# lazytiger/pbrt-rs

Measured on AMD Instinct MI355X. Metric: Mrays/s, higher is better.
Workload: dtype f32

## Files before the change

pbrt-rs_amd/csrc/pbrt_hip.hip:

```cpp
#include <hip/hip_runtime.h>
#include "abi_guard.h"

#include <algorithm>
#include <cstdio>
#include <cstdlib>
#include <cstring>
#include <string>
#include <vector>

#include "host_envmap.h"
#include "host_wide.h"
#include "scene.h"
#include "trace.h"
#include "trace_persistent.h"
#include "trace_wide.h"
#include "trace_stackless.h"

using namespace pb;

static thread_local std::string g_create_error;



extern "C" int pbrt_hip_context_create(int device_id, PbrtHipContext** out) try {
// ... 15 lines not shown
        delete ctx;
        return PBRT_HIP_ERR_DEVICE;
    }
    hipDeviceProp_t prop;
    if (hipGetDeviceProperties(&prop, device_id) != hipSuccess) {
        g_create_error = "hipGetDeviceProperties failed";
        delete ctx;
        return PBRT_HIP_ERR_DEVICE;
    }
    ctx->n_cus = prop.multiProcessorCount;
    ctx->trace_log = std::getenv("PBRT_HIP_TRACE_LOG") != nullptr;
    if (hipStreamCreateWithFlags(&ctx->stream, hipStreamNonBlocking) != hipSuccess ||
        hipEventCreate(&ctx->ev0) != hipSuccess || hipEventCreate(&ctx->ev1) != hipSuccess ||
        hipMalloc((void**)&ctx->d_counters, 8 * sizeof(unsigned long long)) != hipSuccess ||
        hipMalloc((void**)&ctx->d_work_counter, kWorkCounters * sizeof(unsigned int)) != hipSuccess ||
        hipHostMalloc((void**)&ctx->h_counts, 2 * sizeof(unsigned long long), hipHostMallocDefault) != hipSuccess ||
        hipEventCreateWithFlags(&ctx->ev_sync, hipEventDisableTiming) != hipSuccess ||
        hipMemset(ctx->d_counters, 0, 8 * sizeof(unsigned long long)) != hipSuccess) {
        g_create_error = "stream / event creation failed";
        delete ctx;
        return PBRT_HIP_ERR_DEVICE;
    }
    *out = ctx;
    return PBRT_HIP_OK;
}
PB_ABI_CATCH

extern "C" void pbrt_hip_context_destroy(PbrtHipContext* ctx) {
    if (!ctx) return;
    (void)hipSetDevice(ctx->device);
    if (ctx->lost) {
// ... 1355 lines not shown
```

pbrt-rs_amd/csrc/render.hip:

```cpp
#include <hip/hip_runtime.h>
#include "abi_guard.h"

#include <algorithm>
#include <chrono>
#include <cstdio>
#include <cstdlib>
#include <cstring>
#include <string>
#include <thread>
#include <vector>

#include "scene.h"
#include "trace.h"
#include "wavefront.h"

using namespace pb;

extern "C" int pbrt_hip_render_device(PbrtHipScene* s, const PbrtCamera* camera, const PbrtRenderParams* params,
                                      float* d_film, PbrtRenderStats* stats) try {
    if (!s || !camera || !params || !d_film) return PBRT_HIP_ERR_INVALID;
    PB_ENTER(s->ctx);
    HIP_TRY(s->ctx, hipSetDevice(s->ctx->device));
    return wavefront_render(s, *camera, *params, d_film, stats);
}
// ... 650 lines not shown
    ps.two_level = s->d.bvh.instanced ? 1 : 0;
    ps.ray = buf.alloc<float4>(N * 6, &ok);
    ps.hit = buf.alloc<float4>(N * 6, &ok);
    ps.rng = buf.alloc<uint64_t>(N, &ok);
    ps.L = buf.alloc<float4>(N, &ok);
    ps.beta = buf.alloc<float4>(N, &ok);
    ps.nee_a = buf.alloc<float4>(N, &ok);
    ps.nee_f = buf.alloc<float4>(N, &ok);
    ps.nee_b = buf.alloc<float4>(N, &ok);
    ps.nee_light = buf.alloc<int>(N, &ok);
    ps.pfilm = buf.alloc<float2>(N, &ok);
    Queues q[2];
    for (int k = 0; k < 2; ++k) {
        q[k].trace = buf.alloc<uint32_t>(N * 3, &ok);
        q[k].shade = buf.alloc<uint32_t>(N, &ok);
        q[k].counts64 = buf.alloc<unsigned long long>(2, &ok);
        q[k].keys = nullptr;
        for (int a = 0; a < 3; ++a) {
            const float lo = s->d.bvh.root_min[a], hi = s->d.bvh.root_max[a];
            q[k].key_lo[a] = lo;
            q[k].key_inv[a] = hi > lo ? 1.0f / (hi - lo) : 0.0f;
        }
    }
    if (rp.ray_order < 0 || rp.ray_order > 1) return invalid("ray_order must be 0 (Morton order from the second bounce on) or 1 (queue order)");
    const bool sort_rays = rp.ray_order == 0 && rp.integrator == PBRT_INTEGRATOR_PATH;
    constexpr int sort_from = 2;
    uint32_t *sort_keys[2] = {nullptr, nullptr}, *sort_vals = nullptr;
    void* sort_tmp = nullptr;
    size_t sort_tmp_bytes = 0;
    if (sort_rays) {
        sort_keys[0] = buf.alloc<uint32_t>(N * 3, &ok);
// ... 124 lines not shown
    std::memcpy(cam.r2c, camera.raster_to_camera, 64);
    cam.lens_radius = camera.lens_radius;
    cam.focal_distance = camera.focal_distance;
    cam.shutter_open = camera.shutter_open;
    cam.shutter_close = camera.shutter_close;
    cam.kind = camera.kind;
    if (camera.kind < PBRT_CAMERA_PERSPECTIVE || camera.kind > PBRT_CAMERA_ENVIRONMENT) return invalid("unknown camera kind");

    ShadeConsts sc;
    sc.bvh = s->d.bvh;
    sc.materials = s->d.materials;
    sc.lights = s->d.lights;
    sc.n_lights = s->d.n_lights;
    sc.n_infinite = s->d.n_infinite;
    sc.infinite_ids = s->d.infinite_ids;
    sc.env_maps = s->d.env_maps;
    sc.distrib = (rp.light_strategy == 0 || s->d.n_lights == 1) ? s->d.light_distrib_uniform : s->d.light_distrib_power;
    if (rp.integrator == PBRT_INTEGRATOR_PATH && (rp.light_strategy < 0 || rp.light_strategy > 2))
        return invalid("path: light_strategy must be 0 (uniform), 1 (power) or 2 (spatial)");
    std::memcpy(sc.env_cond_func, s->d.env_cond_func, sizeof(sc.env_cond_func));
    std::memcpy(sc.env_cond_cdf, s->d.env_cond_cdf, sizeof(sc.env_cond_cdf));
    std::memcpy(sc.env_cond_int, s->d.env_cond_int, sizeof(sc.env_cond_int));
    std::memcpy(sc.env_marg_func, s->d.env_marg_func, sizeof(sc.env_marg_func));
    std::memcpy(sc.env_marg_cdf, s->d.env_marg_cdf, sizeof(sc.env_marg_cdf));
    sc.env_marg_int = s->d.env_marg_int;
    sc.world_radius = s->d.world_radius;
    sc.light_sample_prefix = d_prefix;
    sc.total_light_samples = prefix.back();
    sc.spatial = nullptr;
    sc.n_voxel[0] = sc.n_voxel[1] = sc.n_voxel[2] = 1;
    sc.mis_bool = ctx->count_traversal != 1 ? 1 : 0;
    if (rp.integrator == PBRT_INTEGRATOR_PATH && rp.light_strategy == 2 && s->d.n_lights > 1) {
        if (!s->d_spatial) {
            const float* mn = s->d.bvh.root_min;
            const float* mx = s->d.bvh.root_max;
            float diag[3] = {mx[0] - mn[0], mx[1] - mn[1], mx[2] - mn[2]};
            int ext = (diag[0] > diag[1] && diag[0] > diag[2]) ? 0 : (diag[1] > diag[2] ? 1 : 2);
            for (int i = 0; i < 3; ++i) s->spatial_voxels[i] = std::max(1, (int)std::round(diag[i] / diag[ext] * 64.0f));
            size_t n_voxels = (size_t)s->spatial_voxels[0] * s->spatial_voxels[1] * s->spatial_voxels[2];
            size_t floats = n_voxels * (size_t)(2 * s->d.n_lights + 2);
            if (floats > (1ull << 30)) return invalid("spatial light distribution: voxels x lights exceed 4 GB; use \"power\"");
            void* p = nullptr;
            HIP_TRY(ctx, hipMalloc(&p, floats * sizeof(float)));
            s->allocs.push_back(p);
            for (int i = 0; i < 3; ++i) sc.n_voxel[i] = s->spatial_voxels[i];
            hipLaunchKernelGGL(k_spatial_light_tables, dim3((unsigned)((n_voxels + 63) / 64)), dim3(64), 0, st, sc, (float*)p);
// ... 134 lines not shown
                    } else if (inst == 2) {
                        if (count_ref) PB_LAUNCH_BINARY(true, 2, false); else PB_LAUNCH_BINARY(false, 2, false);
                    } else if (inst == 1) {
                        if (count_ref) PB_LAUNCH_BINARY(true, 1, false); else PB_LAUNCH_BINARY(false, 1, false);
                    } else {
                        if (count_ref) PB_LAUNCH_BINARY(true, 0, false); else PB_LAUNCH_BINARY(false, 0, false);
                    }
#undef PB_LAUNCH_BINARY
#undef PB_LAUNCH_WIDE
#undef PB_LAUNCH_SPECIAL
                }
                RENDER_TRY(hipGetLastError());
                RENDER_TRY(hipEventRecord(e_t1, st));
            }
            int nxt = cur ^ 1;
            RENDER_TRY(hipMemsetAsync(q[nxt].counts64, 0, 2 * sizeof(unsigned long long), st));
            q[nxt].keys = (sort_rays && wavefront + 1 >= sort_from) ? sort_keys[0] : nullptr;
            if (direct)
{
                dim3 sg((n_shade + 255) / 256), sb(256);
                if (rp.integrator == PBRT_INTEGRATOR_DIRECT && s->glossy)
                    hipLaunchKernelGGL((k_shade_direct<PBRT_INTEGRATOR_DIRECT, true>), sg, sb, 0, st, sc, ps, ds, q[cur], q[nxt], pp, tiles, n_shade);
                else if (rp.integrator == PBRT_INTEGRATOR_DIRECT)
                    hipLaunchKernelGGL((k_shade_direct<PBRT_INTEGRATOR_DIRECT, false>), sg, sb, 0, st, sc, ps, ds, q[cur], q[nxt], pp, tiles, n_shade);
                else if (rp.integrator == PBRT_INTEGRATOR_WHITTED && s->glossy)
                    hipLaunchKernelGGL((k_shade_direct<PBRT_INTEGRATOR_WHITTED, true>), sg, sb, 0, st, sc, ps, ds, q[cur], q[nxt], pp, tiles, n_shade);
                else if (rp.integrator == PBRT_INTEGRATOR_WHITTED)
                    hipLaunchKernelGGL((k_shade_direct<PBRT_INTEGRATOR_WHITTED, false>), sg, sb, 0, st, sc, ps, ds, q[cur], q[nxt], pp, tiles, n_shade);
                else
                    hipLaunchKernelGGL((k_shade_direct<PBRT_INTEGRATOR_AO, false>), sg, sb, 0, st, sc, ps, ds, q[cur], q[nxt], pp, tiles, n_shade);
            }
            else {
                Queues qin = q[cur];
                if (sort_shade && wavefront >= 1 && n_shade >= (1u << 10)) {
                    hipLaunchKernelGGL(k_shade_sort_keys, dim3((n_shade + 255) / 256), dim3(256), 0, st, sc, ps, q[cur].shade, n_shade,
                                       pp.max_depth, shade_keys[0]);
                    size_t tb = shade_tmp_bytes;
                    if (pb::sort_pairs_u32(st, shade_tmp, &tb, shade_keys[0], shade_keys[1], q[cur].shade, shade_sorted, n_shade, 3) != 0 &&
                        rc == PBRT_HIP_OK) {
                        ctx->last_error = "rocPRIM radix sort failed";
                        rc = PBRT_HIP_ERR_DEVICE;
                    }
                    qin.shade = shade_sorted;
                }
                const dim3 sg((n_shade + 255) / 256), sb(256);
                if (bin_shade && wavefront >= 1 && s->glossy)
                    hipLaunchKernelGGL((k_shade<true, true>), sg, sb, 0, st, sc, ps, qin, q[nxt], pp, tiles, n_shade);
                else if (bin_shade && wavefront >= 1)
                    hipLaunchKernelGGL((k_shade<true, false>), sg, sb, 0, st, sc, ps, qin, q[nxt], pp, tiles, n_shade);
                else if (s->glossy)
                    hipLaunchKernelGGL((k_shade<false, true>), sg, sb, 0, st, sc, ps, qin, q[nxt], pp, tiles, n_shade);
                else
                    hipLaunchKernelGGL((k_shade<false, false>), sg, sb, 0, st, sc, ps, qin, q[nxt], pp, tiles, n_shade);
            }
            RENDER_TRY(hipGetLastError());
            RENDER_TRY(hipMemcpyAsync(ctx->h_counts, q[nxt].counts64, sizeof(counts), hipMemcpyDeviceToHost, st));
            RENDER_TRY(hipEventRecord(ctx->ev_sync, st));
            if (rc == PBRT_HIP_OK) {
                hipError_t qe;
                const auto spin_start = std::chrono::steady_clock::now();
                uint32_t polls = 0;
                while ((qe = hipEventQuery(ctx->ev_sync)) == hipErrorNotReady) {
                    if ((++polls & 0xfffu) == 0) {
                        const double waited = std::chrono::duration<double>(std::chrono::steady_clock::now() - spin_start).count();
                        if (waited > ctx->wavefront_deadline_s) {
                            ctx->last_error = "a wavefront did not finish within the deadline (hung kernel?)";
                            ctx->lost = true;
                            rc = PBRT_HIP_ERR_DEVICE;
                            break;
                        }
                        if (waited > 0.05) std::this_thread::yield();
                    }
                }
                if (rc == PBRT_HIP_OK) RENDER_TRY(qe);
            }
            counts[0] = ctx->h_counts[0];
            counts[1] = ctx->h_counts[1];
            if (n_trace > 0 && rc == PBRT_HIP_OK) {
                float ms = 0.0f;
                RENDER_TRY(hipEventElapsedTime(&ms, e_t0, e_t1));
                local.trace_ms += ms;
                local.trace_launches += 1;
                if (ctx->trace_log)
                    std::fprintf(stderr, "[pbrt_hip] k_trace: %u rays %.3f ms (%.0f Mrays/s)\n", n_trace, ms, n_trace / ms * 1e-3);
                ctx->trace_ms += ms;
                ctx->trace_launches += 1;
            }
            {
                uint64_t n_rays = counts[0] & 0xffffffffull, n_shadow = counts[0] >> 32;
                local.rays_closest += n_rays - n_shadow;
                local.rays_shadow += n_shadow;
                counts[0] = n_rays;
            }
            (void)first;
            first = false;
            wavefront += 1;
            cur = nxt;
        }
        if (li_mode) {
            hipLaunchKernelGGL(k_li_output, dim3((unsigned)((li->n + 255) / 256)), dim3(256), 0, st, ps, (uint32_t)li->n, li->d_rgb);
            RENDER_TRY(hipGetLastError());
            continue;
        }
        if (!box) {
            hipLaunchKernelGGL(k_film_splat, dim3((n_paths + 255) / 256), dim3(256), 0, st, ps, pp, tiles, d_film);
            RENDER_TRY(hipGetLastError());
            continue;
// ... 48 lines not shown
```

pbrt-rs_amd/csrc/scene.h:

```cpp
#pragma once
#include <atomic>
#include <hip/hip_runtime.h>

#include <algorithm>
#include <cmath>
#include <cstring>
#include <mutex>
#include <string>
#include <vector>

#include "../../include/pbrt_hip.h"
#include "trace.h"
#include "wide_bvh.h"

#define PB_LOCK(ctx) std::lock_guard<std::recursive_mutex> pb_lock_((ctx)->mu)
#define PB_ENTER(ctx)                                                                                              \
    PB_LOCK(ctx);                                                                                                  \
    if ((ctx)->lost) {                                                                                             \
        (ctx)->last_error = "context lost: an earlier call ran into the wavefront deadline; destroy the context";  \
        return PBRT_HIP_ERR_DEVICE;                                                                                \
    }

struct PbrtHipContext {
    std::recursive_mutex mu;
    int device = 0;
    hipStream_t stream = nullptr;
    hipEvent_t ev0 = nullptr, ev1 = nullptr;
    int n_cus = 0;
    std::string last_error;
    std::atomic<bool> lost{false};
    bool trace_log = false;
    double wavefront_deadline_s = 120.0;
    double trace_ms = 0.0;
    uint64_t trace_launches = 0;
    bool time_trace = true;
    int count_traversal = 0;
// ... 209 lines not shown
```

pbrt-rs_amd/csrc/wf_lights.h:

```cpp
#pragma once
#include "wf_microfacet.h"

namespace pb {

PB_DEV V3 sphere_through(V3 v) {
    return V3{1.0f * v.x + 0.0f * v.y + 0.0f * v.z, 0.0f * v.x + 1.0f * v.y + 0.0f * v.z, 0.0f * v.x + 0.0f * v.y + 1.0f * v.z};
}
PB_DEV float sphere_area(float radius) { return (360.0f * (kPi / 180.0f)) * radius * (radius - (-radius)); }
PB_DEV void sphere_light_sample(float cx, float cy, float cz, float radius, const Surf& sf, float u0, float u1, V3* p_o,
                                V3* err_o, V3* n_o, float* pdf_o) {
    V3 pc = V3{1.0f * 0.0f + 0.0f * 0.0f + 0.0f * 0.0f + cx, 0.0f * 0.0f + 1.0f * 0.0f + 0.0f * 0.0f + cy,
               0.0f * 0.0f + 0.0f * 0.0f + 1.0f * 0.0f + cz};
    V3 p_origin = offset_ray_origin(sf.p, sf.p_error, sf.n, pc - sf.p);
    if (len2(p_origin - pc) <= radius * radius) {
        float z = 1.0f - 2.0f * u0;
        float rr = __builtin_sqrtf(fmaxr(1.0f - z * z, 0.0f));
        float sp, cp;
        det_sincos(2.0f * kPi * u1, &sp, &cp);
        V3 obj = V3{rr * cp, rr * sp, z} * radius;
        V3 n = normalize(sphere_through(obj));
        obj = obj * (radius / length(obj));
        V3 oe = vabs(obj) * kGamma5;
        const float g3 = kGamma3;
        V3 p = V3{1.0f * obj.x + 0.0f * obj.y + 0.0f * obj.z + cx, 0.0f * obj.x + 1.0f * obj.y + 0.0f * obj.z + cy,
// ... 219 lines not shown
    for (int j = 0; j < n; ++j) func[j] = fmaxr(func[j], min_contrib);
    cdf[0] = 0.0f;
    for (int j = 1; j < n + 1; ++j) cdf[j] = cdf[j - 1] + func[j - 1] / (float)n;
    float func_int = cdf[n];
    if (func_int == 0.0f) {
        for (int j = 1; j < n + 1; ++j) cdf[j] = (float)j / (float)n;
    } else {
        for (int j = 1; j < n + 1; ++j) cdf[j] /= func_int;
    }
    func[2 * n + 1] = func_int;
}

template <class Bsdf>
PB_DEV int estimate_direct_emit(const ShadeConsts& sc, const PathState& ps, uint32_t p, const Surf& sf, const Frame& fr,
                                bool nonspecular, const Bsdf& bsdf, int light_num, float ul0, float ul1, float us0, float us1,
                                float pick_pdf, V3 beta) {
    if (!nonspecular) return 0;
    V3 wo = sf.wo;
    DevLight lt = sc.lights[light_num];
    V3 wi, li, p1, p1_err, p1_n;
    float light_pdf;
    light_sample_li(sc, sf, lt, ul0, ul1, &wi, &light_pdf, &li, &p1, &p1_err, &p1_n);
    int nee_flags = 0;
    V3 A = V3{0.0f, 0.0f, 0.0f};
    if (light_pdf > 0.0f && !is_black(li)) {
        V3 f;
        float scattering_pdf;
        bsdf_f_pdf(bsdf, fr, wo, wi, &f, &scattering_pdf);
        f = f * absdot(wi, fr.ns);
        if (!is_black(f)) {
            V3 origin = offset_ray_origin(sf.p, sf.p_error, sf.n, p1 - sf.p);
            V3 target = offset_ray_origin(p1, p1_err, p1_n, origin - p1);
            V3 d = target - origin;
            store_ray(ps, p, RS_SHADOW, origin, d, 1.0f - kShadowEpsilon);
// ... 70 lines not shown
            store_ray(ps, p, RS_MIS, o2, wi2, kInf);
            ps.nee_f[p] = make_float4(f2.x, f2.y, f2.z, weight);
            nee_flags |= PF_NEE_MIS;
            if (sc.mis_bool && lt.type != PBRT_LIGHT_DIFFUSE_AREA) nee_flags |= NEE_MIS_BOOL;
        }
    }
    if (nee_flags) {
        ps.nee_a[p] = make_float4(A.x, A.y, A.z, pick_pdf);
        ps.nee_b[p] = make_float4(beta.x, beta.y, beta.z, spdf);
        ps.nee_light[p] = light_num;
    }
    return nee_flags;
}

PB_DEV V3 estimate_direct_resolve(const ShadeConsts& sc, const PathState& ps, uint32_t p, int flags, float* pick_pdf,
                                  V3* beta_at_vertex) {
    float4 na = ps.nee_a[p], nf = ps.nee_f[p], nb = ps.nee_b[p];
    int light_id = ps.nee_light[p];
    V3 ld = V3{0.0f, 0.0f, 0.0f};
    if (flags & PF_NEE_SHADOW) {
        bool occluded = ps.hit[hit_index(ps, p, RS_SHADOW)].x != 0.0f;
        if (!occluded) ld = ld + V3{na.x, na.y, na.z};
    }
    if (flags & PF_NEE_MIS) {
        int hslot = __float_as_int(ps.hit[hit_index(ps, p, RS_MIS)].x);
        DevLight lt = sc.lights[light_id];
        V3 li = V3{0.0f, 0.0f, 0.0f};
        if (hslot >= 0) {
            int hl = lt.type == PBRT_LIGHT_DIFFUSE_AREA ? (__float_as_int(sc.bvh.tris[3 * (size_t)hslot + 2].w) & kPrimLightMask) - 1 : -2;
            if (hl == light_id) {
                float4 r0 = ps.ray[ray_index(ps, p, RS_MIS)], r1 = ps.ray[ray_index(ps, p, RS_MIS) + 1];
                V3 wi = V3{r0.w, r1.x, r1.y};
                float4 hb = ps.hit[hit_index(ps, p, RS_MIS)];
                V3 n = tri_interaction_normal(sc.bvh, hslot, hb.y, hb.z, hb.w);
                if (lt.two_sided || dot(n, -wi) > 0.0f) li = V3{lt.L[0], lt.L[1], lt.L[2]};
            }
        } else if (lt.type == PBRT_LIGHT_INFINITE) {
            if (lt.slot >= 0) {
                float4 r0 = ps.ray[ray_index(ps, p, RS_MIS)], r1 = ps.ray[ray_index(ps, p, RS_MIS) + 1];
                li = env_le(sc.env_maps[lt.slot], V3{r0.w, r1.x, r1.y});
            } else {
// ... 62 lines not shown
```

pbrt-rs_amd/csrc/wf_path.h:

```cpp
#pragma once
#include "wf_lights.h"

namespace pb {

PB_DEV uint32_t shade_key(const ShadeConsts& sc, const PathState& ps, uint32_t p, int max_depth) {
    int fb = __float_as_int(ps.beta[p].w);
    uint32_t key = 0;
    if ((fb & PF_ALIVE) && (fb >> 8) < max_depth) {
        const size_t hb = hit_index(ps, p, RS_CONT);
        int slot = __float_as_int(ps.hit[hb].x), inst = hit_instance(ps, hb);
        if (slot >= 0) {
            int mat = __float_as_int(sc.bvh.tris[3 * (size_t)slot + 2].z);
            if (sc.bvh.instanced && inst >= 0) {
                int over = __float_as_int(sc.bvh.instances[7 * (size_t)inst + 6].x);
                if (over >= 0) mat = over;
            }
            key = 1u + (uint32_t)sc.materials[mat].type;
        }
    }
    return key;
}
__global__ void k_shade_sort_keys(ShadeConsts sc, PathState ps, const uint32_t* __restrict__ shade_queue, uint32_t n, int max_depth,
                                  uint32_t* __restrict__ keys) {
    uint32_t i = blockIdx.x * blockDim.x + threadIdx.x;
    if (i >= n) return;
    keys[i] = shade_key(sc, ps, shade_queue[i], max_depth);
}

constexpr int shade_keys(bool glossy) { return glossy ? 8 : 6; }
template <int KEYS>
struct ShadeBins {
    uint32_t count[4][KEYS];
    uint32_t path[256];
};

#ifndef PB_SHADE_WAVES
#define PB_SHADE_WAVES 3
#endif
template <bool BIN, bool GLOSSY>
__global__ void __launch_bounds__(256, PB_SHADE_WAVES) k_shade(ShadeConsts sc, PathState ps, Queues qin, Queues qout, PassParams pp,
                                                 TileList tiles, uint32_t n_in) {
    constexpr int kShadeKeys = shade_keys(GLOSSY);
    uint32_t i = blockIdx.x * blockDim.x + threadIdx.x;
    bool active = i < n_in;
    uint32_t p = active ? qin.shade[i] : 0u;
    if (BIN) {
        __shared__ ShadeBins<kShadeKeys> bins;
        const int lane = threadIdx.x & 63, wave = threadIdx.x >> 6;
        const uint32_t key = active ? shade_key(sc, ps, p, pp.max_depth) : (uint32_t)(kShadeKeys - 1);
        uint32_t rank = 0;
#pragma unroll
        for (int k = 0; k < kShadeKeys; ++k) {
            const unsigned long long m = __ballot(key == (uint32_t)k);
            if (key == (uint32_t)k) rank = lane_prefix(m);
            if (lane == 0) bins.count[wave][k] = (uint32_t)__popcll(m);
        }
        __syncthreads();
        uint32_t before = 0;
        for (int k = 0; k < kShadeKeys; ++k)
            for (int w = 0; w < 4; ++w)
                before += ((uint32_t)k < key || ((uint32_t)k == key && w < wave)) ? bins.count[w][k] : 0u;
        bins.path[before + rank] = p;
        uint32_t n_active = 0;
        for (int k = 0; k < kShadeKeys - 1; ++k)
            for (int w = 0; w < 4; ++w) n_active += bins.count[w][k];
        __syncthreads();
        p = bins.path[threadIdx.x];
        active = threadIdx.x < n_active;
    }
    bool emit_cont = false, emit_mis = false, emit_shadow = false, mis_bool = false;

    uint32_t cell = 0;
    if (active) {
        float4 Lq = ps.L[p], bq = ps.beta[p];
        V3 L = V3{Lq.x, Lq.y, Lq.z};
        float eta_scale = Lq.w;
        V3 beta = V3{bq.x, bq.y, bq.z};
        int fb = __float_as_int(bq.w);
        int flags = fb & 0xff, bounces = fb >> 8;
        size_t rbase = ray_index(ps, p, RS_CONT), hbase = hit_index(ps, p, RS_CONT);

        if (flags & (PF_NEE_SHADOW | PF_NEE_MIS)) {
            float pick_pdf;
            V3 beta_v;
            V3 ld = estimate_direct_resolve(sc, ps, p, flags, &pick_pdf, &beta_v);
            ld = ld / pick_pdf;
            L = L + mulv(beta_v, ld);
            flags &= ~(PF_NEE_SHADOW | PF_NEE_MIS);
        }

        if (flags & PF_ALIVE) {
            flags &= ~PF_ALIVE;
            float4 r0 = ps.ray[rbase], r1 = ps.ray[rbase + 1];
            V3 rd = V3{r0.w, r1.x, r1.y};
            float4 h0 = ps.hit[hbase];
            int hslot = __float_as_int(h0.x);
            bool found = hslot >= 0;
            Surf sf;
            if (found) {
                sf = surface_from_hit(sc.bvh, hslot, hit_instance(ps, hbase), h0.y, h0.z, h0.w, rd);
                if (qout.keys) cell = ray_sort_cell(sf.p.x, sf.p.y, sf.p.z, qout.key_lo, qout.key_inv);
            }
            if (bounces == 0 || (flags & PF_SPECULAR_BOUNCE)) {
                if (found) {
                    L = L + mulv(beta, surface_le(sc, sf, -rd));
                } else {
                    for (int k = 0; k < sc.n_infinite; ++k) {
                        DevLight lt = sc.lights[sc.infinite_ids[k]];
                        V3 le = lt.slot >= 0 ? env_le(sc.env_maps[lt.slot], rd) : V3{lt.L[0], lt.L[1], lt.L[2]};
                        L = L + mulv(beta, le);
                    }
                }
            }
            if (found && bounces < pp.max_depth) {
                DevMaterial mat = sc.materials[sf.material];
                Samp sm = path_sampler(ps, pp, tiles, p);
                if (mat.type == PBRT_MAT_NONE) {
                    V3 o = offset_ray_origin(sf.p, sf.p_error, sf.n, rd);
                    store_ray(ps, p, RS_CONT, o, rd, kInf);
                    flags |= PF_ALIVE;
                    emit_cont = true;
                } else {
                    Frame fr = make_frame(sf);
                    V3 kd = V3{mat.kd[0], mat.kd[1], mat.kd[2]};
                    V3 kt = V3{mat.kt[0], mat.kt[1], mat.kt[2]};
                    V3 wo = -rd;
                    bool has_lobe;
                    bool nonspecular;
                    NsBsdf nsb;
                    if (GLOSSY) {
                        nsb = ns_bsdf(mat);
                        nonspecular = nsb.n > 0;
                        if (mat.type == PBRT_MAT_GLASS) has_lobe = !(is_black(kd) && is_black(kt));
                        else if (mat.type == PBRT_MAT_MIRROR) has_lobe = !is_black(kd);
                        else has_lobe = nonspecular;
                    } else {
                        if (mat.type == PBRT_MAT_GLASS) has_lobe = !(is_black(kd) && is_black(kt));
                        else has_lobe = !is_black(kd);
                        nonspecular = (mat.type == PBRT_MAT_MATTE) && has_lobe;
                    }

                    if (nonspecular && sc.n_lights > 0) {
                        float u_pick = samp_1d(pp, sm);
                        DevDistribution1D distrib = light_distribution_lookup(sc, sf.p);
                        int light_num = find_interval_cdf(distrib.cdf, distrib.n + 1, u_pick);
                        float pick_pdf = distrib.func_int > 0.0f ? distrib.func[light_num] / (distrib.func_int * (float)distrib.n)
                                                                 : 0.0f;
                        if (pick_pdf != 0.0f) {
                            float ul0, ul1, us0, us1;
                            samp_2d(pp, sm, &ul0, &ul1);
                            samp_2d(pp, sm, &us0, &us1);
                            int nee_flags = GLOSSY ? estimate_direct_emit(sc, ps, p, sf, fr, true, nsb, light_num, ul0, ul1, us0,
                                                                          us1, pick_pdf, beta)
                                                   : estimate_direct_emit(sc, ps, p, sf, fr, true, MatteBsdf{kd}, light_num, ul0, ul1,
                                                                          us0, us1, pick_pdf, beta);
                            flags |= nee_flags & 0xff;
                            emit_shadow = (nee_flags & PF_NEE_SHADOW) != 0;
                            emit_mis = (nee_flags & PF_NEE_MIS) != 0;
                            mis_bool = (nee_flags & NEE_MIS_BOOL) != 0;
                        }
                    }

                    float u0 = 0.0f, u1 = 0.0f;
                    samp_2d(pp, sm, &u0, &u1);
                    V3 wi = V3{0.0f, 0.0f, 0.0f}, f = V3{0.0f, 0.0f, 0.0f};
                    float pdf = 0.0f;
                    bool sampled_specular = false, sampled_transmission = false;
                    if (has_lobe) {
                        if (GLOSSY && nonspecular) {
                            bool ok;
// ... 19 lines not shown
                        beta = mulv(beta, f * (absdot(wi, fr.ns) / pdf));
                        flags = (flags & ~PF_SPECULAR_BOUNCE) | (sampled_specular ? PF_SPECULAR_BOUNCE : 0);
                        if (sampled_specular && sampled_transmission) {
                            float eta = mat.eta;
                            eta_scale *= (dot(wo, sf.n) > 0.0f) ? (eta * eta) : 1.0f / (eta * eta);
                        }
                        V3 o = offset_ray_origin(sf.p, sf.p_error, sf.n, wi);
                        bool alive = true;
                        V3 rr_beta = beta * eta_scale;
                        if (max_comp(rr_beta) < pp.rr_threshold && bounces > 3) {
                            float qq = fmaxr(0.05f, 1.0f - max_comp(rr_beta));
                            if (samp_1d(pp, sm) < qq) alive = false;
                            else beta = beta / (1.0f - qq);
                        }
                        if (alive) {
                            store_ray(ps, p, RS_CONT, o, wi, kInf);
                            flags |= PF_ALIVE;
                            emit_cont = true;
                            bounces += 1;
                        }
                    }
                }
                samp_store(ps, p, sm);
            }
        }
        ps.L[p] = make_float4(L.x, L.y, L.z, eta_scale);
        ps.beta[p] = make_float4(beta.x, beta.y, beta.z, __int_as_float((bounces << 8) | flags));
    }

    __shared__ BlockAppend sh;
    const bool again = emit_cont || emit_mis || emit_shadow;
    block_append(sh, qout, p, emit_cont, emit_mis, emit_shadow, again, cell, mis_bool);
}

}
```

pbrt-rs_amd/csrc/wf_state.h:

```cpp
#pragma once
#include <hip/hip_runtime.h>

#include "scene.h"
#include "trace.h"
#include "trace_persistent.h"
#include "trace_wide.h"
#include "trace_stackless.h"

namespace pb {

constexpr int kTile = 16;
enum PathFlags : int {
    PF_SPECULAR_BOUNCE = 1,
    PF_ALIVE = 2,
    PF_NEE_SHADOW = 4,
    PF_NEE_MIS = 8,
    PF_VALID = 16,
};
enum RaySlot : int { RS_CONT = 0, RS_MIS = 1, RS_SHADOW = 2 };
constexpr uint32_t RS_MIS_BOOL = 3;
constexpr int NEE_MIS_BOOL = 0x100;

struct PathState {
    float4* ray;
// ... 93 lines not shown
    uint32_t q[3] = {(uint32_t)fminf(fmaxf(fx * kCells, 0.0f), kCells - 1.0f), (uint32_t)fminf(fmaxf(fy * kCells, 0.0f), kCells - 1.0f),
                     (uint32_t)fminf(fmaxf(fz * kCells, 0.0f), kCells - 1.0f)};
    uint32_t code = 0;
    for (int b = 0; b < PB_SORT_AXIS_BITS; ++b)
        for (int k = 0; k < 3; ++k) code |= ((q[k] >> b) & 1u) << (3 * b + k);
    return code;
}

PB_DEV int64_t pixel_number(const PassParams& pp, int x, int y) {
    return (int64_t)(y - pp.sb_y0) * pp.sb_w + (x - pp.sb_x0);
}
PB_DEV uint64_t sample_sequence(const PassParams& pp, int x, int y, int s) {
    return pp.seed ^ (uint64_t)(pixel_number(pp, x, y) * (int64_t)pp.spp + s);
}

struct BlockAppend {
    uint32_t wave_rays[16];
    uint32_t wave_shadow[16];
    uint32_t wave_paths[16];
    uint32_t base_rays, base_paths;
};
PB_DEV uint32_t lane_prefix(unsigned long long mask) {
    return __builtin_amdgcn_mbcnt_hi((uint32_t)(mask >> 32), __builtin_amdgcn_mbcnt_lo((uint32_t)mask, 0));
}
PB_DEV void block_append(BlockAppend& sh, const Queues& q, uint32_t p, bool cont, bool mis, bool shadow, bool again,
                         uint32_t cell = 0, bool mis_bool = false) {
    const int lane = threadIdx.x & 63, wave = threadIdx.x >> 6, n_waves = (blockDim.x + 63) >> 6;
    unsigned long long mc = __ballot(cont), mm = __ballot(mis), ms = __ballot(shadow), ma = __ballot(again);
    uint32_t wc = (uint32_t)__popcll(mc), wm = (uint32_t)__popcll(mm), ws = (uint32_t)__popcll(ms);
    if (lane == 0) {
        sh.wave_rays[wave] = wc + wm + ws;
        sh.wave_shadow[wave] = ws;
        sh.wave_paths[wave] = (uint32_t)__popcll(ma);
    }
    __syncthreads();
    if (threadIdx.x == 0) {
        uint32_t tr = 0, tsd = 0, tp = 0;
        for (int w = 0; w < n_waves; ++w) {
            uint32_t r = sh.wave_rays[w], pth = sh.wave_paths[w];
            sh.wave_rays[w] = tr;
            sh.wave_paths[w] = tp;
            tr += r;
            tsd += sh.wave_shadow[w];
            tp += pth;
        }
        unsigned long long old = 0;
        if (tr) old = atomicAdd(&q.counts64[0], (unsigned long long)tr | ((unsigned long long)tsd << 32));
        sh.base_rays = (uint32_t)old;
        sh.base_paths = tp ? (uint32_t)atomicAdd(&q.counts64[1], (unsigned long long)tp) : 0u;
    }
    __syncthreads();
    uint32_t rbase = sh.base_rays + sh.wave_rays[wave];
    uint32_t ic = rbase + lane_prefix(mc), im = rbase + wc + lane_prefix(mm), is = rbase + wc + wm + lane_prefix(ms);
    if (cont) q.trace[ic] = p * 4u + RS_CONT;
    if (mis) q.trace[im] = p * 4u + (mis_bool ? RS_MIS_BOOL : (uint32_t)RS_MIS);
    if (shadow) q.trace[is] = p * 4u + RS_SHADOW;
    if (q.keys) {
        if (cont) q.keys[ic] = cell;
        if (mis) q.keys[im] = mis_bool ? (cell | (1u << (kSortKeyBits - 1))) : cell;
        if (shadow) q.keys[is] = cell | (1u << (kSortKeyBits - 1));
    }
    if (again) q.shade[sh.base_paths + sh.wave_paths[wave] + lane_prefix(ma)] = p;
}

PB_DEV void store_ray(const PathState& ps, uint32_t p, int slot, V3 o, V3 d, float tmax) {
    size_t i = ray_index(ps, p, slot);
    ps.ray[i] = make_float4(o.x, o.y, o.z, d.x);
    ps.ray[i + 1] = make_float4(d.y, d.z, tmax, 0.0f);
}

struct DevCamera {
    float c2w[16], r2c[16];
    float lens_radius, focal_distance, shutter_open, shutter_close;
    int kind;
};
PB_DEV V3 xform_point(const float* m, V3 p) {
    float xp = m[0] * p.x + m[1] * p.y + m[2] * p.z + m[3];
// ... 18 lines not shown
```

pbrt-rs_amd/csrc/wf_surface.h:

```cpp
#pragma once
#include "wf_generate_trace.h"

namespace pb {

struct Surf {
    V3 p, p_error, n, dpdu, wo;
    V3 ns, sdpdu;
    int material, light;
};

PB_DEV void tri_vertices(const DevBVH& bvh, int slot, V3* p0, V3* p1, V3* p2, int* prim, int* mat, int* light) {
    float4 a = bvh.tris[3 * (size_t)slot], b = bvh.tris[3 * (size_t)slot + 1], c = bvh.tris[3 * (size_t)slot + 2];
    *p0 = V3{a.x, a.y, a.z};
    *p1 = V3{a.w, b.x, b.y};
    *p2 = V3{b.z, b.w, c.x};
    *prim = __float_as_int(c.y);
    *mat = __float_as_int(c.z);
    *light = (__float_as_int(c.w) & kPrimLightMask) - 1;
}

PB_DEV void tri_shading_geometry(const DevBVH& bvh, int slot, V3 p0, V3 p1, V3 p2, float b0, float b1, float b2, V3* n_out,
                                 V3* ns_out, V3* dpdu_out, V3* sdpdu_out) {
    float uv0x = 0.0f, uv0y = 0.0f, uv1x = 1.0f, uv1y = 0.0f, uv2x = 1.0f, uv2y = 1.0f;
    float4 s0 = make_float4(0, 0, 0, 0), s1 = s0, s2 = s0, s3 = s0, s4 = s0;
// ... 262 lines not shown
    DevBVH bvh;
    const DevMaterial* materials;
    const DevLight* lights;
    int n_lights, n_infinite;
    const int* infinite_ids;
    const DevEnvMap* env_maps;
    DevDistribution1D distrib;
    float env_cond_func[2][2], env_cond_cdf[2][3], env_cond_int[2];
    float env_marg_func[2], env_marg_cdf[3], env_marg_int;
    float world_radius;
    const int* light_sample_prefix;
    int total_light_samples;
    const float* spatial;
    int n_voxel[3];
    int mis_bool;
};

PB_DEV V3 env_lookup(const DevEnvMap& e, float st_s, float st_t) {
    float s = st_s * (float)e.w - 0.5f, t = st_t * (float)e.h - 0.5f;
    if (!(s >= -1.0f && s <= (float)e.w)) s = -0.5f;
    if (!(t >= -1.0f && t <= (float)e.h)) t = -0.5f;
    float fs = __builtin_floorf(s), ft = __builtin_floorf(t);
    float ds = s - fs, dt = t - ft;
    int s0 = (int)fs, t0 = (int)ft;
    s0 = s0 < 0 ? s0 + e.w : (s0 >= e.w ? s0 - e.w : s0);
    t0 = t0 < 0 ? t0 + e.h : (t0 >= e.h ? t0 - e.h : t0);
    int s1 = s0 + 1 >= e.w ? s0 + 1 - e.w : s0 + 1;
    int t1 = t0 + 1 >= e.h ? t0 + 1 - e.h : t0 + 1;
    float4 a = e.texels[(size_t)t0 * e.w + s0], b = e.texels[(size_t)t1 * e.w + s0];
    float4 c = e.texels[(size_t)t0 * e.w + s1], d = e.texels[(size_t)t1 * e.w + s1];
    float wa = (1.0f - ds) * (1.0f - dt), wb = (1.0f - ds) * dt, wc = ds * (1.0f - dt), wd = ds * dt;
// ... 88 lines not shown
    sm.dim2 = (c >> 10) & 0x3f;
    sm.arr = (c >> 16) & 0xffff;
    sm.h_offset = pp.smp.kind == PBRT_SAMPLER_HALTON ? halton_pixel_offset(pp.smp, x, y) : 0;
    return sm;
}

PB_DEV Frame make_frame(const Surf& sf) {
    Frame fr;
    fr.ns = sf.ns;
    fr.ng = sf.n;
    fr.ss = normalize(sf.sdpdu);
    fr.ts = cross(fr.ns, fr.ss);
    return fr;
}

PB_DEV V3 surface_le(const ShadeConsts& sc, const Surf& sf, V3 w) {
    if (sf.light >= 0) {
        DevLight lt = sc.lights[sf.light];
        if (lt.two_sided || dot(sf.n, w) > 0.0f) return V3{lt.L[0], lt.L[1], lt.L[2]};
    }
    return V3{0.0f, 0.0f, 0.0f};
}

}
```

Measured before the change: 2856.

## Stage shade lookup tables in LDS and restructure queue append reservation

The shade kernel now copies the lights, materials, light distribution func/cdf and infinite-light ids into a per-block LDS table when they fit in 2048 words. Material, light and CDF lookups then read from LDS instead of global memory. Queue append is split into reserve and commit so the block reserves its queue slots before it writes its path state. The single atomic now packs the ray and path counts, and the shadow tally moves to a separate cache line. The costs are the LDS fill and an extra __syncthreads per block, plus LDS pressure that may reduce occupancy.

Measured after the change: 2866 (median of 4 runs). Within noise of the previous version (+0.3%).

```diff
diff --git a/pbrt-rs_amd/csrc/pbrt_hip.hip b/pbrt-rs_amd/csrc/pbrt_hip.hip
--- a/pbrt-rs_amd/csrc/pbrt_hip.hip
+++ b/pbrt-rs_amd/csrc/pbrt_hip.hip
@@ -53,7 +53,7 @@
         hipEventCreate(&ctx->ev0) != hipSuccess || hipEventCreate(&ctx->ev1) != hipSuccess ||
         hipMalloc((void**)&ctx->d_counters, 8 * sizeof(unsigned long long)) != hipSuccess ||
         hipMalloc((void**)&ctx->d_work_counter, kWorkCounters * sizeof(unsigned int)) != hipSuccess ||
-        hipHostMalloc((void**)&ctx->h_counts, 2 * sizeof(unsigned long long), hipHostMallocDefault) != hipSuccess ||
+        hipHostMalloc((void**)&ctx->h_counts, pb::kQueueCountWords * sizeof(unsigned long long), hipHostMallocDefault) != hipSuccess ||
         hipEventCreateWithFlags(&ctx->ev_sync, hipEventDisableTiming) != hipSuccess ||
         hipMemset(ctx->d_counters, 0, 8 * sizeof(unsigned long long)) != hipSuccess) {
         g_create_error = "stream / event creation failed";
diff --git a/pbrt-rs_amd/csrc/render.hip b/pbrt-rs_amd/csrc/render.hip
--- a/pbrt-rs_amd/csrc/render.hip
+++ b/pbrt-rs_amd/csrc/render.hip
@@ -688,7 +688,7 @@
     for (int k = 0; k < 2; ++k) {
         q[k].trace = buf.alloc<uint32_t>(N * 3, &ok);
         q[k].shade = buf.alloc<uint32_t>(N, &ok);
-        q[k].counts64 = buf.alloc<unsigned long long>(2, &ok);
+        q[k].counts64 = buf.alloc<unsigned long long>(kQueueCountWords, &ok);
         q[k].keys = nullptr;
         for (int a = 0; a < 3; ++a) {
             const float lo = s->d.bvh.root_min[a], hi = s->d.bvh.root_max[a];
@@ -843,6 +843,7 @@
     sc.n_lights = s->d.n_lights;
     sc.n_infinite = s->d.n_infinite;
     sc.infinite_ids = s->d.infinite_ids;
+    sc.n_materials = s->d.n_materials;
     sc.env_maps = s->d.env_maps;
     sc.distrib = (rp.light_strategy == 0 || s->d.n_lights == 1) ? s->d.light_distrib_uniform : s->d.light_distrib_power;
     if (rp.integrator == PBRT_INTEGRATOR_PATH && (rp.light_strategy < 0 || rp.light_strategy > 2))
@@ -859,6 +860,7 @@
     sc.spatial = nullptr;
     sc.n_voxel[0] = sc.n_voxel[1] = sc.n_voxel[2] = 1;
     sc.mis_bool = ctx->count_traversal != 1 ? 1 : 0;
+    shade_tab_layout(&sc);
     if (rp.integrator == PBRT_INTEGRATOR_PATH && rp.light_strategy == 2 && s->d.n_lights > 1) {
         if (!s->d_spatial) {
             const float* mn = s->d.bvh.root_min;
@@ -1023,7 +1025,7 @@
                 RENDER_TRY(hipEventRecord(e_t1, st));
             }
             int nxt = cur ^ 1;
-            RENDER_TRY(hipMemsetAsync(q[nxt].counts64, 0, 2 * sizeof(unsigned long long), st));
+            RENDER_TRY(hipMemsetAsync(q[nxt].counts64, 0, kQueueCountWords * sizeof(unsigned long long), st));
             q[nxt].keys = (sort_rays && wavefront + 1 >= sort_from) ? sort_keys[0] : nullptr;
             if (direct)
 {
@@ -1053,17 +1055,25 @@
                     qin.shade = shade_sorted;
                 }
                 const dim3 sg((n_shade + 255) / 256), sb(256);
+#define PB_LAUNCH_SHADE(BIN, GLOSSY)                                                                                \
+    do {                                                                                                            \
+        if (sc.tab_off[4] > 0)                                                                                      \
+            hipLaunchKernelGGL((k_shade<BIN, GLOSSY, true>), sg, sb, 0, st, sc, ps, qin, q[nxt], pp, tiles, n_shade);  \
+        else                                                                                                        \
+            hipLaunchKernelGGL((k_shade<BIN, GLOSSY, false>), sg, sb, 0, st, sc, ps, qin, q[nxt], pp, tiles, n_shade); \
+    } while (0)
                 if (bin_shade && wavefront >= 1 && s->glossy)
-                    hipLaunchKernelGGL((k_shade<true, true>), sg, sb, 0, st, sc, ps, qin, q[nxt], pp, tiles, n_shade);
+                    PB_LAUNCH_SHADE(true, true);
                 else if (bin_shade && wavefront >= 1)
-                    hipLaunchKernelGGL((k_shade<true, false>), sg, sb, 0, st, sc, ps, qin, q[nxt], pp, tiles, n_shade);
+                    PB_LAUNCH_SHADE(true, false);
                 else if (s->glossy)
-                    hipLaunchKernelGGL((k_shade<false, true>), sg, sb, 0, st, sc, ps, qin, q[nxt], pp, tiles, n_shade);
+                    PB_LAUNCH_SHADE(false, true);
                 else
-                    hipLaunchKernelGGL((k_shade<false, false>), sg, sb, 0, st, sc, ps, qin, q[nxt], pp, tiles, n_shade);
+                    PB_LAUNCH_SHADE(false, false);
+#undef PB_LAUNCH_SHADE
             }
             RENDER_TRY(hipGetLastError());
-            RENDER_TRY(hipMemcpyAsync(ctx->h_counts, q[nxt].counts64, sizeof(counts), hipMemcpyDeviceToHost, st));
+            RENDER_TRY(hipMemcpyAsync(ctx->h_counts, q[nxt].counts64, kQueueCountWords * sizeof(unsigned long long), hipMemcpyDeviceToHost, st));
             RENDER_TRY(hipEventRecord(ctx->ev_sync, st));
             if (rc == PBRT_HIP_OK) {
                 hipError_t qe;
@@ -1083,8 +1093,14 @@
                 }
                 if (rc == PBRT_HIP_OK) RENDER_TRY(qe);
             }
-            counts[0] = ctx->h_counts[0];
+#if PB_APPEND_TWO_ATOMICS
+            counts[0] = ctx->h_counts[0] & 0xffffffffull;
             counts[1] = ctx->h_counts[1];
+#else
+            counts[0] = ctx->h_counts[0] & 0xffffffffull;
+            counts[1] = ctx->h_counts[0] >> 32;
+#endif
+            const uint64_t n_shadow_next = ctx->h_counts[kShadowTallyWord];
             if (n_trace > 0 && rc == PBRT_HIP_OK) {
                 float ms = 0.0f;
                 RENDER_TRY(hipEventElapsedTime(&ms, e_t0, e_t1));
@@ -1096,10 +1112,9 @@
                 ctx->trace_launches += 1;
             }
             {
-                uint64_t n_rays = counts[0] & 0xffffffffull, n_shadow = counts[0] >> 32;
+                const uint64_t n_rays = counts[0], n_shadow = n_shadow_next;
                 local.rays_closest += n_rays - n_shadow;
                 local.rays_shadow += n_shadow;
-                counts[0] = n_rays;
             }
             (void)first;
             first = false;
diff --git a/pbrt-rs_amd/csrc/scene.h b/pbrt-rs_amd/csrc/scene.h
--- a/pbrt-rs_amd/csrc/scene.h
+++ b/pbrt-rs_amd/csrc/scene.h
@@ -20,6 +20,11 @@
         (ctx)->last_error = "context lost: an earlier call ran into the wavefront deadline; destroy the context";  \
         return PBRT_HIP_ERR_DEVICE;                                                                                \
     }
+
+namespace pb {
+constexpr int kShadowTallyWord = 16;
+constexpr int kQueueCountWords = kShadowTallyWord + 1;
+}
 
 struct PbrtHipContext {
     std::recursive_mutex mu;
diff --git a/pbrt-rs_amd/csrc/wf_lights.h b/pbrt-rs_amd/csrc/wf_lights.h
--- a/pbrt-rs_amd/csrc/wf_lights.h
+++ b/pbrt-rs_amd/csrc/wf_lights.h
@@ -257,10 +257,10 @@
 template <class Bsdf>
 PB_DEV int estimate_direct_emit(const ShadeConsts& sc, const PathState& ps, uint32_t p, const Surf& sf, const Frame& fr,
                                 bool nonspecular, const Bsdf& bsdf, int light_num, float ul0, float ul1, float us0, float us1,
-                                float pick_pdf, V3 beta) {
+                                float pick_pdf, V3 beta, const ShadeTab& tab = ShadeTab{}) {
     if (!nonspecular) return 0;
     V3 wo = sf.wo;
-    DevLight lt = sc.lights[light_num];
+    DevLight lt = shade_light(sc, tab, light_num);
     V3 wi, li, p1, p1_err, p1_n;
     float light_pdf;
     light_sample_li(sc, sf, lt, ul0, ul1, &wi, &light_pdf, &li, &p1, &p1_err, &p1_n);
@@ -361,7 +361,7 @@
 }
 
 PB_DEV V3 estimate_direct_resolve(const ShadeConsts& sc, const PathState& ps, uint32_t p, int flags, float* pick_pdf,
-                                  V3* beta_at_vertex) {
+                                  V3* beta_at_vertex, const ShadeTab& tab = ShadeTab{}) {
     float4 na = ps.nee_a[p], nf = ps.nee_f[p], nb = ps.nee_b[p];
     int light_id = ps.nee_light[p];
     V3 ld = V3{0.0f, 0.0f, 0.0f};
@@ -371,7 +371,7 @@
     }
     if (flags & PF_NEE_MIS) {
         int hslot = __float_as_int(ps.hit[hit_index(ps, p, RS_MIS)].x);
-        DevLight lt = sc.lights[light_id];
+        DevLight lt = shade_light(sc, tab, light_id);
         V3 li = V3{0.0f, 0.0f, 0.0f};
         if (hslot >= 0) {
             int hl = lt.type == PBRT_LIGHT_DIFFUSE_AREA ? (__float_as_int(sc.bvh.tris[3 * (size_t)hslot + 2].w) & kPrimLightMask) - 1 : -2;
diff --git a/pbrt-rs_amd/csrc/wf_path.h b/pbrt-rs_amd/csrc/wf_path.h
--- a/pbrt-rs_amd/csrc/wf_path.h
+++ b/pbrt-rs_amd/csrc/wf_path.h
@@ -37,13 +37,28 @@
 #ifndef PB_SHADE_WAVES
 #define PB_SHADE_WAVES 3
 #endif
-template <bool BIN, bool GLOSSY>
+#ifndef PB_SHADE_EARLY_RESERVE
+#define PB_SHADE_EARLY_RESERVE 1
+#endif
+template <bool BIN, bool GLOSSY, bool TAB>
 __global__ void __launch_bounds__(256, PB_SHADE_WAVES) k_shade(ShadeConsts sc, PathState ps, Queues qin, Queues qout, PassParams pp,
                                                  TileList tiles, uint32_t n_in) {
     constexpr int kShadeKeys = shade_keys(GLOSSY);
     uint32_t i = blockIdx.x * blockDim.x + threadIdx.x;
     bool active = i < n_in;
     uint32_t p = active ? qin.shade[i] : 0u;
+    __shared__ uint32_t tab_words[TAB ? kShadeTabWords : 1];
+    PB_LDS uint32_t* const tab_lds = (PB_LDS uint32_t*)tab_words;
+    if (TAB) shade_tab_fill(sc, tab_lds);
+    const ShadeTab tab = shade_tab_view(sc, tab_lds, TAB);
+    float4 Lq = make_float4(0.0f, 0.0f, 0.0f, 0.0f), bq = Lq;
+    if (!BIN) {
+        if (active) {
+            Lq = ps.L[p];
+            bq = ps.beta[p];
+        }
+        if (TAB) __syncthreads();
+    }
     if (BIN) {
         __shared__ ShadeBins<kShadeKeys> bins;
         const int lane = threadIdx.x & 63, wave = threadIdx.x >> 6;
@@ -67,23 +82,30 @@
         __syncthreads();
         p = bins.path[threadIdx.x];
         active = threadIdx.x < n_active;
+        if (active) {
+            Lq = ps.L[p];
+            bq = ps.beta[p];
+        }
     }
     bool emit_cont = false, emit_mis = false, emit_shadow = false, mis_bool = false;
 
     uint32_t cell = 0;
+    V3 L = V3{Lq.x, Lq.y, Lq.z}, beta = V3{bq.x, bq.y, bq.z};
+    float eta_scale = Lq.w;
+    int flags = 0, bounces = 0;
+    V3 cont_o = V3{0.0f, 0.0f, 0.0f}, cont_d = cont_o;
+    bool store_samp = false;
+    uint64_t samp_rng = 0;
+    int samp_dims = 0;
     if (active) {
-        float4 Lq = ps.L[p], bq = ps.beta[p];
-        V3 L = V3{Lq.x, Lq.y, Lq.z};
-        float eta_scale = Lq.w;
-        V3 beta = V3{bq.x, bq.y, bq.z};
         int fb = __float_as_int(bq.w);
-        int flags = fb & 0xff, bounces = fb >> 8;
+        flags = fb & 0xff, bounces = fb >> 8;
         size_t rbase = ray_index(ps, p, RS_CONT), hbase = hit_index(ps, p, RS_CONT);
 
         if (flags & (PF_NEE_SHADOW | PF_NEE_MIS)) {
             float pick_pdf;
             V3 beta_v;
-            V3 ld = estimate_direct_resolve(sc, ps, p, flags, &pick_pdf, &beta_v);
+            V3 ld = estimate_direct_resolve(sc, ps, p, flags, &pick_pdf, &beta_v, tab);
             ld = ld / pick_pdf;
             L = L + mulv(beta_v, ld);
             flags &= ~(PF_NEE_SHADOW | PF_NEE_MIS);
@@ -103,21 +125,21 @@
             }
             if (bounces == 0 || (flags & PF_SPECULAR_BOUNCE)) {
                 if (found) {
-                    L = L + mulv(beta, surface_le(sc, sf, -rd));
+                    L = L + mulv(beta, surface_le(sc, sf, -rd, tab));
                 } else {
                     for (int k = 0; k < sc.n_infinite; ++k) {
-                        DevLight lt = sc.lights[sc.infinite_ids[k]];
+                        DevLight lt = shade_light(sc, tab, shade_infinite_id(sc, tab, k));
                         V3 le = lt.slot >= 0 ? env_le(sc.env_maps[lt.slot], rd) : V3{lt.L[0], lt.L[1], lt.L[2]};
                         L = L + mulv(beta, le);
                     }
                 }
             }
             if (found && bounces < pp.max_depth) {
-                DevMaterial mat = sc.materials[sf.material];
+                DevMaterial mat = shade_material(sc, tab, sf.material);
                 Samp sm = path_sampler(ps, pp, tiles, p);
                 if (mat.type == PBRT_MAT_NONE) {
-                    V3 o = offset_ray_origin(sf.p, sf.p_error, sf.n, rd);
-                    store_ray(ps, p, RS_CONT, o, rd, kInf);
+                    cont_o = offset_ray_origin(sf.p, sf.p_error, sf.n, rd);
+                    cont_d = rd;
                     flags |= PF_ALIVE;
                     emit_cont = true;
                 } else {
@@ -143,17 +165,17 @@
                     if (nonspecular && sc.n_lights > 0) {
                         float u_pick = samp_1d(pp, sm);
                         DevDistribution1D distrib = light_distribution_lookup(sc, sf.p);
-                        int light_num = find_interval_cdf(distrib.cdf, distrib.n + 1, u_pick);
-                        float pick_pdf = distrib.func_int > 0.0f ? distrib.func[light_num] / (distrib.func_int * (float)distrib.n)
+                        int light_num = find_interval_pick(sc, tab, distrib, u_pick);
+                        float pick_pdf = distrib.func_int > 0.0f ? pick_func(sc, tab, distrib, light_num) / (distrib.func_int * (float)distrib.n)
                                                                  : 0.0f;
                         if (pick_pdf != 0.0f) {
                             float ul0, ul1, us0, us1;
                             samp_2d(pp, sm, &ul0, &ul1);
                             samp_2d(pp, sm, &us0, &us1);
                             int nee_flags = GLOSSY ? estimate_direct_emit(sc, ps, p, sf, fr, true, nsb, light_num, ul0, ul1, us0,
-                                                                          us1, pick_pdf, beta)
+                                                                          us1, pick_pdf, beta, tab)
                                                    : estimate_direct_emit(sc, ps, p, sf, fr, true, MatteBsdf{kd}, light_num, ul0, ul1,
-                                                                          us0, us1, pick_pdf, beta);
+                                                                          us0, us1, pick_pdf, beta, tab);
                             flags |= nee_flags & 0xff;
                             emit_shadow = (nee_flags & PF_NEE_SHADOW) != 0;
                             emit_mis = (nee_flags & PF_NEE_MIS) != 0;
@@ -203,23 +225,39 @@
                             else beta = beta / (1.0f - qq);
                         }
                         if (alive) {
-                            store_ray(ps, p, RS_CONT, o, wi, kInf);
+                            cont_o = o;
+                            cont_d = wi;
                             flags |= PF_ALIVE;
                             emit_cont = true;
                             bounces += 1;
                         }
                     }
                 }
-                samp_store(ps, p, sm);
-            }
+                store_samp = true;
+                samp_rng = sm.rng.state;
+                samp_dims = sm.dim1 | (sm.dim2 << 10) | (sm.arr << 16);
+            }
+        }
+    }
+
+    __shared__ BlockAppend sh;
+    const bool again = emit_cont || emit_mis || emit_shadow;
+#if PB_SHADE_EARLY_RESERVE
+    const AppendTicket ticket = block_reserve(sh, qout, emit_cont, emit_mis, emit_shadow, again);
+#endif
+    if (active) {
+        if (emit_cont) store_ray(ps, p, RS_CONT, cont_o, cont_d, kInf);
+        if (store_samp) {
+            ps.rng[p] = samp_rng;
+            ps.samp[p] = samp_dims;
         }
         ps.L[p] = make_float4(L.x, L.y, L.z, eta_scale);
         ps.beta[p] = make_float4(beta.x, beta.y, beta.z, __int_as_float((bounces << 8) | flags));
     }
-
-    __shared__ BlockAppend sh;
-    const bool again = emit_cont || emit_mis || emit_shadow;
-    block_append(sh, qout, p, emit_cont, emit_mis, emit_shadow, again, cell, mis_bool);
-}
-
-}
+#if !PB_SHADE_EARLY_RESERVE
+    const AppendTicket ticket = block_reserve(sh, qout, emit_cont, emit_mis, emit_shadow, again);
+#endif
+    block_commit(sh, qout, ticket, p, emit_cont, emit_mis, emit_shadow, again, cell, mis_bool);
+}
+
+}
diff --git a/pbrt-rs_amd/csrc/wf_state.h b/pbrt-rs_amd/csrc/wf_state.h
--- a/pbrt-rs_amd/csrc/wf_state.h
+++ b/pbrt-rs_amd/csrc/wf_state.h
@@ -131,27 +131,41 @@
     return pp.seed ^ (uint64_t)(pixel_number(pp, x, y) * (int64_t)pp.spp + s);
 }
 
+#ifndef PB_APPEND_TWO_ATOMICS
+#define PB_APPEND_TWO_ATOMICS 0
+#endif
+static_assert(kShadowTallyWord * sizeof(unsigned long long) >= 128, "the shadow tally must not share the reservation word's cache line");
 struct BlockAppend {
     uint32_t wave_rays[16];
     uint32_t wave_shadow[16];
     uint32_t wave_paths[16];
     uint32_t base_rays, base_paths;
 };
+struct AppendTicket {
+    unsigned long long mc, mm, ms, ma;
+    unsigned long long old;
+};
 PB_DEV uint32_t lane_prefix(unsigned long long mask) {
     return __builtin_amdgcn_mbcnt_hi((uint32_t)(mask >> 32), __builtin_amdgcn_mbcnt_lo((uint32_t)mask, 0));
 }
-PB_DEV void block_append(BlockAppend& sh, const Queues& q, uint32_t p, bool cont, bool mis, bool shadow, bool again,
-                         uint32_t cell = 0, bool mis_bool = false) {
+PB_DEV AppendTicket block_reserve(BlockAppend& sh, const Queues& q, bool cont, bool mis, bool shadow, bool again) {
     const int lane = threadIdx.x & 63, wave = threadIdx.x >> 6, n_waves = (blockDim.x + 63) >> 6;
-    unsigned long long mc = __ballot(cont), mm = __ballot(mis), ms = __ballot(shadow), ma = __ballot(again);
-    uint32_t wc = (uint32_t)__popcll(mc), wm = (uint32_t)__popcll(mm), ws = (uint32_t)__popcll(ms);
+    AppendTicket t;
+    t.mc = __ballot(cont), t.mm = __ballot(mis), t.ms = __ballot(shadow), t.ma = __ballot(again);
+    t.old = 0;
+    uint32_t ws = (uint32_t)__popcll(t.ms);
     if (lane == 0) {
-        sh.wave_rays[wave] = wc + wm + ws;
+        sh.wave_rays[wave] = (uint32_t)__popcll(t.mc) + (uint32_t)__popcll(t.mm) + ws;
         sh.wave_shadow[wave] = ws;
-        sh.wave_paths[wave] = (uint32_t)__popcll(ma);
+        sh.wave_paths[wave] = (uint32_t)__popcll(t.ma);
     }
     __syncthreads();
     if (threadIdx.x == 0) {
+        uint32_t opaque_zero = 0;
+#if defined(__HIP_DEVICE_COMPILE__)
+        asm volatile("" : "+v"(opaque_zero));
+#endif
+        unsigned long long* const counts = q.counts64 + opaque_zero;
         uint32_t tr = 0, tsd = 0, tp = 0;
         for (int w = 0; w < n_waves; ++w) {
             uint32_t r = sh.wave_rays[w], pth = sh.wave_paths[w];
@@ -161,14 +175,28 @@
             tsd += sh.wave_shadow[w];
             tp += pth;
         }
-        unsigned long long old = 0;
-        if (tr) old = atomicAdd(&q.counts64[0], (unsigned long long)tr | ((unsigned long long)tsd << 32));
-        sh.base_rays = (uint32_t)old;
-        sh.base_paths = tp ? (uint32_t)atomicAdd(&q.counts64[1], (unsigned long long)tp) : 0u;
+#if PB_APPEND_TWO_ATOMICS
+        unsigned long long lo = tr ? atomicAdd(&counts[0], (unsigned long long)tr) : 0ull;
+        unsigned long long hi = tp ? atomicAdd(&counts[1], (unsigned long long)tp) : 0ull;
+        t.old = (lo & 0xffffffffull) | (hi << 32);
+#else
+        if (tr | tp) t.old = atomicAdd(&counts[0], (unsigned long long)tr | ((unsigned long long)tp << 32));
+#endif
+        if (tsd) (void)atomicAdd(&counts[kShadowTallyWord], (unsigned long long)tsd);
+    }
+    return t;
+}
+PB_DEV void block_commit(BlockAppend& sh, const Queues& q, const AppendTicket& t, uint32_t p, bool cont, bool mis, bool shadow,
+                         bool again, uint32_t cell = 0, bool mis_bool = false) {
+    const int wave = threadIdx.x >> 6;
+    if (threadIdx.x == 0) {
+        sh.base_rays = (uint32_t)t.old;
+        sh.base_paths = (uint32_t)(t.old >> 32);
     }
     __syncthreads();
+    const uint32_t wc = (uint32_t)__popcll(t.mc), wm = (uint32_t)__popcll(t.mm);
     uint32_t rbase = sh.base_rays + sh.wave_rays[wave];
-    uint32_t ic = rbase + lane_prefix(mc), im = rbase + wc + lane_prefix(mm), is = rbase + wc + wm + lane_prefix(ms);
+    uint32_t ic = rbase + lane_prefix(t.mc), im = rbase + wc + lane_prefix(t.mm), is = rbase + wc + wm + lane_prefix(t.ms);
     if (cont) q.trace[ic] = p * 4u + RS_CONT;
     if (mis) q.trace[im] = p * 4u + (mis_bool ? RS_MIS_BOOL : (uint32_t)RS_MIS);
     if (shadow) q.trace[is] = p * 4u + RS_SHADOW;
@@ -177,7 +205,12 @@
         if (mis) q.keys[im] = mis_bool ? (cell | (1u << (kSortKeyBits - 1))) : cell;
         if (shadow) q.keys[is] = cell | (1u << (kSortKeyBits - 1));
     }
-    if (again) q.shade[sh.base_paths + sh.wave_paths[wave] + lane_prefix(ma)] = p;
+    if (again) q.shade[sh.base_paths + sh.wave_paths[wave] + lane_prefix(t.ma)] = p;
+}
+PB_DEV void block_append(BlockAppend& sh, const Queues& q, uint32_t p, bool cont, bool mis, bool shadow, bool again,
+                         uint32_t cell = 0, bool mis_bool = false) {
+    const AppendTicket t = block_reserve(sh, q, cont, mis, shadow, again);
+    block_commit(sh, q, t, p, cont, mis, shadow, again, cell, mis_bool);
 }
 
 PB_DEV void store_ray(const PathState& ps, uint32_t p, int slot, V3 o, V3 d, float tmax) {
diff --git a/pbrt-rs_amd/csrc/wf_surface.h b/pbrt-rs_amd/csrc/wf_surface.h
--- a/pbrt-rs_amd/csrc/wf_surface.h
+++ b/pbrt-rs_amd/csrc/wf_surface.h
@@ -300,7 +300,96 @@
     const float* spatial;
     int n_voxel[3];
     int mis_bool;
+    int n_materials;
+    int tab_off[5];
 };
+
+#ifndef PB_SHADE_LDS_TABLES
+#define PB_SHADE_LDS_TABLES 1
+#endif
+constexpr int kShadeTabWords = 2048;
+constexpr int kLightWords = (int)(sizeof(DevLight) / 4), kMaterialWords = (int)(sizeof(DevMaterial) / 4);
+static_assert(sizeof(DevLight) % 4 == 0 && sizeof(DevMaterial) % 4 == 0 && alignof(DevLight) == 4 && alignof(DevMaterial) == 4,
+              "the tables are copied and read back as 4-byte words");
+#if defined(__HIP_DEVICE_COMPILE__)
+#define PB_LDS __attribute__((address_space(3)))
+#else
+#define PB_LDS
+#endif
+struct ShadeTab {
+    const PB_LDS uint32_t* w = nullptr;
+    int on = 0;
+    int distrib = 0;
+};
+inline void shade_tab_layout(ShadeConsts* sc) {
+    const bool have_distrib = sc->distrib.func && sc->distrib.cdf && sc->distrib.n > 0;
+    const long long n_func = have_distrib ? sc->distrib.n : 0, n_cdf = have_distrib ? sc->distrib.n + 1 : 0;
+    long long off = (long long)sc->n_lights * kLightWords;
+    long long o[5];
+    o[0] = off, off += (long long)sc->n_materials * kMaterialWords;
+    o[1] = off, off += n_func;
+    o[2] = off, off += n_cdf;
+    o[3] = off, off += sc->n_infinite;
+    o[4] = off;
+    const bool fits = PB_SHADE_LDS_TABLES && off <= kShadeTabWords && sc->n_materials > 0;
+    for (int k = 0; k < 5; ++k) sc->tab_off[k] = fits ? (int)o[k] : 0;
+}
+PB_DEV void shade_tab_fill(const ShadeConsts& sc, PB_LDS uint32_t* tab) {
+    const uint32_t* lights = (const uint32_t*)sc.lights;
+    const uint32_t* materials = (const uint32_t*)sc.materials;
+    const uint32_t* func = (const uint32_t*)sc.distrib.func;
+    const uint32_t* cdf = (const uint32_t*)sc.distrib.cdf;
+    const uint32_t* inf = (const uint32_t*)sc.infinite_ids;
+    const int total = sc.tab_off[4] < kShadeTabWords ? sc.tab_off[4] : kShadeTabWords;
+    for (int w = (int)threadIdx.x; w < total; w += (int)blockDim.x) {
+        const uint32_t* src = w < sc.tab_off[0]   ? lights + w
+                              : w < sc.tab_off[1] ? materials + (w - sc.tab_off[0])
+                              : w < sc.tab_off[2] ? func + (w - sc.tab_off[1])
+                              : w < sc.tab_off[3] ? cdf + (w - sc.tab_off[2])
+                                                  : inf + (w - sc.tab_off[3]);
+        tab[w] = *src;
+    }
+}
+PB_DEV ShadeTab shade_tab_view(const ShadeConsts& sc, const PB_LDS uint32_t* tab, bool on) {
+    ShadeTab t;
+    t.w = tab;
+    t.on = on;
+    t.distrib = t.on && !sc.spatial && sc.tab_off[2] > sc.tab_off[1];
+    return t;
+}
+PB_DEV DevLight shade_light(const ShadeConsts& sc, const ShadeTab& t, int i) {
+    if (t.on) return ((const PB_LDS DevLight*)t.w)[i];
+    return sc.lights[i];
+}
+PB_DEV DevMaterial shade_material(const ShadeConsts& sc, const ShadeTab& t, int i) {
+    if (t.on) return ((const PB_LDS DevMaterial*)(t.w + sc.tab_off[0]))[i];
+    return sc.materials[i];
+}
+PB_DEV int shade_infinite_id(const ShadeConsts& sc, const ShadeTab& t, int k) {
+    if (t.on) return (int)t.w[sc.tab_off[3] + k];
+    return sc.infinite_ids[k];
+}
+PB_DEV int find_interval_pick(const ShadeConsts& sc, const ShadeTab& t, const DevDistribution1D& d, float u) {
+    if (!t.distrib) return find_interval_cdf(d.cdf, d.n + 1, u);
+    const PB_LDS float* cdf = (const PB_LDS float*)(t.w + sc.tab_off[2]);
+    const int size = d.n + 1;
+    int first = 0, len = size;
+    while (len > 0) {
+        int half = len >> 1, middle = first + half;
+        if (cdf[middle] < u) {
+            first = middle + 1;
+            len -= half + 1;
+        } else {
+            len = half;
+        }
+    }
+    int v = first - 1;
+    return v < 0 ? 0 : (v > size - 2 ? size - 2 : v);
+}
+PB_DEV float pick_func(const ShadeConsts& sc, const ShadeTab& t, const DevDistribution1D& d, int i) {
+    if (t.distrib) return ((const PB_LDS float*)(t.w + sc.tab_off[1]))[i];
+    return d.func[i];
+}
 
 PB_DEV V3 env_lookup(const DevEnvMap& e, float st_s, float st_t) {
     float s = st_s * (float)e.w - 0.5f, t = st_t * (float)e.h - 0.5f;
@@ -419,9 +508,9 @@
     return fr;
 }
 
-PB_DEV V3 surface_le(const ShadeConsts& sc, const Surf& sf, V3 w) {
+PB_DEV V3 surface_le(const ShadeConsts& sc, const Surf& sf, V3 w, const ShadeTab& tab = ShadeTab{}) {
     if (sf.light >= 0) {
-        DevLight lt = sc.lights[sf.light];
+        DevLight lt = shade_light(sc, tab, sf.light);
         if (lt.two_sided || dot(sf.n, w) > 0.0f) return V3{lt.L[0], lt.L[1], lt.L[2]};
     }
     return V3{0.0f, 0.0f, 0.0f};
```
